# AllenInstitute/distributed-vae

Measured on AMD Instinct MI355X. Metric: cells/sec per train step (fwd+loss+bwd+opt), higher is better.
Workload: dtype f32; 1 GPU; cpl_mixVAE A=2 arms, synthetic-10x-v1 50000 cells x 5000 genes per GPU, batch 5000/GPU, fp32, H=100 L=10 C=92 S=2, x_drop=0.5, Adam lr=1e-3; global_batch=5000, parallelism=dp1, noise=in-kernel Philox4x32-10

## Files before the change

### distributed-vae_amd/_native.py

```python
from __future__ import annotations

import ctypes as C
import os
from typing import Dict, Optional

import torch

HERE = os.path.dirname(os.path.abspath(__file__))
LIB_PATH = os.environ.get("MMVAE_LIB") or os.path.join(HERE, "libmmvae_hip.so")

ABI_VERSION = 5
N_PARAM_TENSORS = 28
N_BN = 6
MAX_ARMS = 8

PARAM_NAMES = [
    "fc1.weight", "fc1.bias", "fc2.weight", "fc2.bias", "fc3.weight", "fc3.bias", "fc4.weight", "fc4.bias",
    "fc5.weight", "fc5.bias", "fcc.weight", "fcc.bias", "fc_mu.weight", "fc_sigma.weight", "fc_mu.bias",
    "fc_sigma.bias", "fc6.weight", "fc6.bias", "fc7.weight", "fc7.bias", "fc8.weight", "fc8.bias",
    "fc9.weight", "fc9.bias", "fc10.weight", "fc10.bias", "fc11.weight", "fc11.bias",
]
BN_NAMES = ["batch_l1", "batch_l2", "batch_l3", "batch_l4", "batch_l5", "batch_s"]

WS_IDS = {name: i for i, name in enumerate([
# ... 81 lines not shown
    "fc11": ("FC11_GENERAL", "FC11_ZG", "FC11_ZT", "FC11_BF16", "FC11_X3", "FC11_OUT_BF16", "FC11_OUT_X3"),
    "zero": ("ZERO_NONE", "ZERO_MEMSET", "ZERO_XBITS", "ZERO_PRESPLIT"),
    "couple": ("COUPLE_INLINE", "COUPLE_SIDE", "COUPLE_IN_DEC"),
}


def debug_plan(dims: "Dims", hyper: "Hyper", ex: Optional["Exec"], kind: str, params_align: int = 16, x_align: int = 16,
               x_arm_stride: int = 0, has_x16: bool = False, fc11_grad: bool = True) -> Dict[str, object]:
    out = (C.c_int32 * PLAN_FIELDS)()
    check(lib().mmvae_debug_plan(C.byref(dims), C.byref(hyper), C.byref(ex) if ex is not None else None, CALL_KINDS[kind],
                                 int(params_align), int(x_align), int(x_arm_stride), int(bool(has_x16)), int(bool(fc11_grad)),
                                 C.byref(out)), "mmvae_debug_plan")
    plan = {}
    for name, v in zip(PLAN_NAMES, out):
        if name in PLAN_ENUMS:
            plan[name] = PLAN_ENUMS[name][v]
        elif name == "kind":
            plan[name] = next(k for k, i in CALL_KINDS.items() if i == v)
        elif name in ("gd10_slabs", "dw11_slabs"):
            plan[name] = int(v)
        else:
            plan[name] = bool(v)
    return plan


_lib = None


def lib():
    global _lib
    if _lib is not None:
        return _lib
    if not os.path.exists(LIB_PATH):
        raise NativeError(
            f"{LIB_PATH} not found: build the HIP extension first "
            "(python -c 'import __graft_entry__ as g; g.build()' or python distributed-vae_amd/build.py). "
            "There is no CPU fallback.")
    L = C.CDLL(LIB_PATH)
    vp, i64, f32, i32 = C.c_void_p, C.c_int64, C.c_float, C.c_int
    L.mmvae_abi_version.restype = C.c_int
    L.mmvae_last_error_string.restype = C.c_char_p
    L.mmvae_check_dims.argtypes = [C.POINTER(Dims)]
    L.mmvae_param_layout.argtypes = [C.POINTER(Dims), C.POINTER(ParamLayout)]
    ex = C.POINTER(Exec)
    L.mmvae_workspace_bytes.argtypes = [C.POINTER(Dims), ex]
    L.mmvae_workspace_bytes.restype = C.c_size_t
    L.mmvae_ws_offset.argtypes = [C.POINTER(Dims), ex, C.c_int]
    L.mmvae_ws_offset.restype = i64
    L.mmvae_splits.argtypes = [C.POINTER(Dims), ex, C.POINTER(C.c_int32 * 6)]
    L.mmvae_forward.argtypes = [C.POINTER(Dims), C.POINTER(Hyper), C.POINTER(Noise), vp, vp, vp, vp, i64, vp, i32,
                                vp, C.c_size_t, ex, vp]
    L.mmvae_loss.argtypes = [C.POINTER(Dims), C.POINTER(Hyper), vp, C.c_size_t, vp, ex, vp]
    L.mmvae_backward.argtypes = [C.POINTER(Dims), C.POINTER(Hyper), C.POINTER(Noise), vp, vp, i64, f32, vp,
                                 C.c_size_t, vp, ex, vp]
    L.mmvae_adam_step.argtypes = [i64, vp, vp, vp, vp, i64, f32, f32, f32, f32, f32, i32, vp]
    L.mmvae_train_step.argtypes = [C.POINTER(Dims), C.POINTER(Hyper), C.POINTER(Noise), vp, vp, vp, vp, i64, vp,
                                   C.c_size_t, vp, vp, i32, vp, vp, i64, f32, f32, f32, f32, f32, i32, ex, vp]
    L.mmvae_train_step_rows.argtypes = [C.POINTER(Dims), C.POINTER(Hyper), C.POINTER(Noise), vp, vp, vp, vp, vp, i64, i64, vp, vp,
                                        C.c_size_t, vp, vp, i32, vp, vp, i64, f32, f32, f32, f32, f32, i32, ex, vp]
    L.mmvae_train_step_rows.restype = C.c_int
    L.mmvae_to_bf16.argtypes = [vp, i64, i64, i32, vp, vp]
    L.mmvae_to_bf16.restype = C.c_int
    L.mmvae_debug_stage.argtypes = [C.POINTER(Dims), C.POINTER(Hyper), C.POINTER(Noise), i32, vp, vp, i64, vp,
                                    C.c_size_t, vp, ex, vp]
    L.mmvae_dump_noise.argtypes = [C.POINTER(Dims), C.POINTER(Hyper), C.POINTER(Noise), vp, vp, vp, vp, vp]
    L.mmvae_debug_plan.argtypes = [C.POINTER(Dims), C.POINTER(Hyper), ex, i32, i32, i32, i64, i32, i32,
                                   C.POINTER(C.c_int32 * PLAN_FIELDS)]
    L.mmvae_debug_plan.restype = C.c_int
    L.mmvae_eval_classify.argtypes = [C.POINTER(Dims), C.POINTER(Hyper), vp, vp, vp, i64, vp, C.c_size_t, vp, vp, ex,
                                      vp]
    L.mmvae_classify.argtypes = [vp, i64, i32, vp, vp]
    L.mmvae_confmat_accumulate.argtypes = [vp, i32, i64, i32, vp, vp]
    L.mmvae_consensus.argtypes = [vp, i32, i32, vp, vp, vp]
    L.mmvae_aug_packed_floats.argtypes = [C.POINTER(AugDims)]
    L.mmvae_aug_packed_floats.restype = C.c_size_t
    L.mmvae_aug_workspace_bytes.argtypes = [C.POINTER(AugDims), i32]
    L.mmvae_aug_workspace_bytes.restype = C.c_size_t
    L.mmvae_aug_pack.argtypes = [C.POINTER(AugDims), C.POINTER(AugTensors), vp, vp]
    L.mmvae_augment.argtypes = [C.POINTER(AugDims), vp, vp, i64, vp, vp, f32, vp, C.c_size_t, vp, vp, i32, ex, vp]
    L.mmvae_gather_rows.argtypes = [vp, i64, i64, vp, i64, i32, vp, vp]
    L.mmvae_tp_planes_bytes.argtypes = [i64, i32, i32]
    L.mmvae_tp_planes_bytes.restype = C.c_size_t
    L.mmvae_tp_planes.argtypes = [vp, i64, i64, i32, i32, vp, vp]
    L.mmvae_augment_rows.argtypes = [C.POINTER(AugDims), vp, vp, i64, i32, vp, vp, vp, f32, vp, C.c_size_t, vp, vp, i32, ex, vp]
    L.mmvae_decode_workspace_bytes.argtypes = [C.POINTER(Dims), ex]
    L.mmvae_decode_workspace_bytes.restype = C.c_size_t
    L.mmvae_decode.argtypes = [C.POINTER(Dims), C.POINTER(Hyper), vp, vp, i64, vp, i64, vp, vp, C.c_size_t, ex, vp]
    L.mmvae_decode.restype = C.c_int
    L.mmvae_state_changes_workspace_bytes.argtypes = [C.POINTER(Dims), i32, ex]
    L.mmvae_state_changes_workspace_bytes.restype = C.c_size_t
    L.mmvae_state_changes.argtypes = [C.POINTER(Dims), C.POINTER(Hyper), C.POINTER(Noise), vp, vp, vp, i32, i32, vp, vp,
# ... 330 lines not shown
```

### distributed-vae_amd/csrc/api.hip

```cpp
#include "common.hpp"
#include <stdarg.h>
#include <stdio.h>
#include <string.h>

namespace mmvae {

static thread_local char g_err[512] = "";
void set_error(const char* fmt, ...) {
    va_list ap;
    va_start(ap, fmt);
    vsnprintf(g_err, sizeof(g_err), fmt, ap);
    va_end(ap);
}

Splits default_splits(const mmvae_dims& d, const mmvae_exec* ex) {
    int g_split[6] = {0, 0, 0, 0, 0, 0};
    if (ex) for (int i = 0; i < 6; ++i) g_split[i] = ex->split[i] > 0 && ex->split[i] <= 64 ? ex->split[i] : 0;
    constexpr int CUS = 256;
    auto fit = [](int base_blocks, int slots, int cap) {
        const int base = base_blocks > 0 ? base_blocks : 1;
        auto eff = [&](int k) { const int n = base * k; return (double)n / (double)(((n + slots - 1) / slots) * slots); };
        int pick = 1;
        double best = 0.0;
        for (int k = 1; k <= cap; ++k) {
// ... 19 lines not shown
    s.ks_small = g_split[3] > 0 ? g_split[3] : fit(N_SMALL * d.A, 3 * CUS, 32);
    s.ks_small = min(s.ks_small, max(1, cdiv(d.B, 32)));
    s.ks_gd10 = g_split[4] > 0 ? g_split[4] : fit(nb128 * d.A, (fastdims && d.H == 100 ? 2 : 3) * CUS, 16);
    if (g_split[4] <= 0 && fastdims && d.H == 100) {
        const int wg = cdiv(d.B, 256) * d.A;
        int best = s.ks_gd10;
        double best_eff = 0.0;
        for (int ks = 1; ks <= 16; ++ks) {
            const int n = wg * ks;
            const double eff = (double)n / (double)(cdiv(n, CUS) * CUS);
            if (eff > best_eff + 0.02) { best_eff = eff; best = ks; }
            if (eff >= 0.93) { best = ks; break; }
        }
        s.ks_gd10 = best;
    }
    s.ks_gd10 = min(s.ks_gd10, max(1, cdiv(d.D, fastdims && d.H == 100 ? 64 : 32)));
    if (ex && ex->tune[MMVAE_TUNE_ENGINE] == 2 && fastdims && x3_fc11_fits(d)) {
        const int pairs_b = cdiv(nb128, 2), pairs_d = cdiv(cdiv(d.D, 128), 2);
        if (g_split[0] <= 0) s.ks_fc1 = min(fit(pairs_b * d.A, CUS, 16), max(1, cdiv(d.D, 32)));
        if (g_split[4] <= 0) s.ks_gd10 = min(fit(nb128 * d.A, CUS, 16), max(1, cdiv(d.D, 64)));
        if (g_split[2] <= 0) s.ks_dw = min(fit(pairs_d * d.A, CUS, 16), max(1, cdiv(d.B, 32)));
        if (g_split[5] <= 0) {
            const int nwg = max(1, pairs_d * d.A);
            const bool chain_x3 = chain_planes_fit(d) && !ex->tune[MMVAE_TUNE_CHAIN_FP32];
            const int target = chain_x3 ? 140 : 3 * CUS / 8;
            s.ks_dw11 = min(max(1, (target + nwg / 2) / nwg), max(1, cdiv(d.B, 32)));
        }
        if (g_split[3] <= 0) s.ks_small = min(fit(cdiv(N_SMALL * d.A, 2), CUS, 32), max(1, cdiv(d.B, 32)));
    }
    if (ex && ex->tune[MMVAE_TUNE_ENGINE] == 1 && fastdims && bf16_tiles_fit(d)) {
        if (g_split[3] <= 0) s.ks_small = min(fit(cdiv(N_SMALL * d.A, 2), CUS, 32), max(1, cdiv(d.B, 32)));
        if (g_split[5] <= 0) {
            const int nwg = max(1, cdiv(d.D, 128) * d.A);
            s.ks_dw11 = min(max(1, (5 * CUS / 8 + nwg / 2) / nwg), max(1, cdiv(d.B, 32)));
        }
    }
    return s;
}

POff make_poff(const mmvae_dims& d) {
    POff p{};
    const int64_t D = d.D, H = d.H, L = d.L, C = d.C, S = d.S;
    const int64_t sizes[MMVAE_N_PARAM_TENSORS] = {
        H * D, H, H * H, H, H * H, H, H * H, H, L * H, L, C * L, C, S * (L + C), S * (L + C), S, S,
        L * (C + S), L, H * L, H, H * H, H, H * H, H, H * H, H, D * H, D};
    int64_t off = 0;
    for (int t = 0; t < MMVAE_N_PARAM_TENSORS; ++t) {
// ... 152 lines not shown
static void make_plan(Ctx& c, CallKind kind, const float* params, const float* x, int64_t xs, bool fc11_grad = true) {
    const mmvae_dims& d = c.d;
    const mmvae_hyper& h = c.h;
    const Layout& L = c.lay;
    Plan& p = c.plan;
    p = Plan{};
    p.kind = kind;
    const bool step = kind == CALL_STEP || kind == CALL_STEP_ROWS, fwd = step || kind == CALL_FORWARD || kind == CALL_CLASSIFY ||
                                                                 kind == CALL_TRAVERSE;
    const bool dropout = c.dropout(), side = c.side() != nullptr;
    p.fast = fast_dims(d) && al16(params) && al16(x) && (xs & 3) == 0 && d.H >= 4 && (int64_t)d.B * d.D < ((int64_t)1 << 30);
    const bool bf16_tiles = (h.gemm_bf16 == 1 || h.gemm_bf16 == 2) && bf16_tiles_fit(d);
    const bool x3 = h.gemm_bf16 == 2 && bf16_tiles_fit(d);
    p.big = !p.fast ? GEMM_GENERAL : x3 ? GEMM_X3 : bf16_tiles ? GEMM_BF16 : GEMM_FP32;
    p.small_x3 = bf16_tiles;
    const bool slots = fc11_slots_fit(L, d.B);
    if (!p.fast) p.fc11 = FC11_GENERAL;
    else if (p.big == GEMM_X3 && fc11_grad && x3_fc11_fits(d) && slots) p.fc11 = FC11_X3;
    else if (p.big == GEMM_BF16) p.fc11 = FC11_BF16;
    else if (fc11_grad && d.H == 100 && (int64_t)cdiv(d.B, 256) * L.sp.ks_gd10 <= L.n11) p.fc11 = FC11_ZG;
    else p.fc11 = FC11_ZT;
    p.gd10_slabs = p.fast ? L.sp.ks_gd10 : L.sp.ns_fc11;
    p.dw11_slabs = p.fast ? L.sp.ks_dw11 : L.sp.ks_dw;
    p.chain_planes = p.fast && bf16_tiles && chain_planes_fit(d) && !c.tune(MMVAE_TUNE_CHAIN_FP32);
    p.lat_half = d.C <= 32 * LH_CPL && d.L <= 32 && 2 * d.S <= 32;
    p.narrow = h.gemm_bf16 == 1 && c.x16 != nullptr && bf16_tiles_fit(d) && (d.D & 7) == 0;
    p.presplit = fwd && p.fast && (x3 || p.chain_planes);
    p.bwd_small_planes = kind == CALL_BACKWARD && p.chain_planes;
    p.d10_planes = x3;
    p.dz1_in_apply = (x3 || p.narrow) && (d.H & 1) == 0;
    if (fwd && h.training) p.zero = p.presplit && dropout ? ZERO_PRESPLIT : p.fast && dropout ? ZERO_XBITS : ZERO_MEMSET;
    p.rowmap = kind == CALL_STEP_ROWS && p.zero == ZERO_PRESPLIT && slots && (p.fc11 == FC11_X3 || p.fc11 == FC11_BF16);
    p.dz11_bf16 = p.rowmap && c.x16 != nullptr && p.fc11 == FC11_BF16;
    p.dw11_side = (step || kind == CALL_BACKWARD) && p.fast && side;
    p.loss_on_side = step && p.fast && side;
    const int cs = c.tune(MMVAE_TUNE_COUPLE_SIDE);
    const bool role = p.loss_on_side && c.use_acc() && p.chain_planes && d.A >= 2 && d.A <= 5 && cs != 1 && (d.A >= 4 || cs == 3);
    p.couple = step && side ? (role ? COUPLE_IN_DEC : COUPLE_SIDE) : COUPLE_INLINE;
    p.lat_fork_rides = p.couple == COUPLE_SIDE && p.lat_half;
    p.fc11_fork_rides = p.loss_on_side && (p.fc11 == FC11_X3 || p.fc11 == FC11_BF16);
    if (kind == CALL_DECODE) {
        if (!p.fast) p.fc11 = FC11_GENERAL;
        else if (p.big == GEMM_X3 && x3_fc11_fits(d)) p.fc11 = FC11_OUT_X3;
        else if (p.big == GEMM_BF16) p.fc11 = FC11_OUT_BF16;
        else p.fc11 = FC11_ZT;
        p.d10_planes = p.fc11 == FC11_OUT_X3 || p.fc11 == FC11_OUT_BF16;
        p.dec_planes = p.d10_planes || p.chain_planes;
    }
}

static int fork_to_side(const Ctx& c, int ev, bool rode = false) {
// ... 456 lines not shown
            if (!fast) return launch_dw_big(c, nz, x, x_arm_stride);
            if (int rc = dw1(c, x, x_arm_stride)) return rc;
            return dw11(c);
        case 9: return launch_make_xbits(c, nz);
        case 20: return launch_chain_fwd_enc(c, 3, params, nullptr, nullptr);
        case 21: return launch_chain_bwd_enc(c, 3, params);
        case 10: case 11: case 12: case 13: case 14:
            if (!fast) { set_error("stage %d needs the fast path", stage); return MMVAE_E_UNSUPPORTED; }
            if (stage == 10) return fc11_main(c, params, x, x_arm_stride, nullptr, 1);
            if (stage == 11) return fc11_gd10(c, params, nullptr, 1);
            if (stage == 12) return dw1(c, x, x_arm_stride);
            if (stage == 13) return dw11(c);
            return fc1_gemm(c, params, x, x_arm_stride);
        case 3: return launch_dw_small(c);
        case 4: return launch_chain_fwd_dec(c, params);
        case 5: return launch_chain_bwd_dec(c, params);
        case 6: return launch_lat_fwd(c, nz, params, nullptr, nullptr);
        case 7: return launch_lat_bwd(c, nz, params);
        case 8: if (!grads) { set_error("grads is null"); return MMVAE_E_BADARG; } return launch_reduce_grads(c, grads, 1.f, nullptr);
        default: set_error("unknown stage %d", stage); return MMVAE_E_BADARG;
    }
}

int mmvae_debug_plan(const mmvae_dims* d, const mmvae_hyper* h, const mmvae_exec* ex, int call_kind, int params_align,
                     int x_align, int64_t x_arm_stride, int has_x16, int fc11_grad, int32_t out[MMVAE_PLAN_FIELDS]) {
    if (int rc = check_dims(d)) return rc;
    if (!h || !out) { set_error("null hyper / out"); return MMVAE_E_BADARG; }
    if (int rc = check_gemm_engine(h->gemm_bf16)) return rc;
    static_assert(MMVAE_CALL_STEP == CALL_STEP && MMVAE_CALL_STEP_ROWS == CALL_STEP_ROWS && MMVAE_CALL_FORWARD == CALL_FORWARD &&
                  MMVAE_CALL_BACKWARD == CALL_BACKWARD && MMVAE_CALL_LOSS == CALL_LOSS && MMVAE_CALL_CLASSIFY == CALL_CLASSIFY &&
                  MMVAE_CALL_REPLAY == CALL_REPLAY && MMVAE_CALL_DECODE == CALL_DECODE && MMVAE_CALL_TRAVERSE == CALL_TRAVERSE,
                  "MMVAE_CALL_* (include/mmvae.h) are the values of CallKind");
    if (call_kind < CALL_STEP || call_kind > CALL_TRAVERSE) { set_error("unknown call kind %d", call_kind); return MMVAE_E_BADARG; }
    if (params_align < 0 || x_align < 0) { set_error("negative alignment"); return MMVAE_E_BADARG; }
    Ctx c{};
    c.d = *d;
    c.h = *h;
    if (call_kind == CALL_DECODE || call_kind == CALL_TRAVERSE || call_kind == CALL_CLASSIFY) c.h.training = 0;
    if (ex) c.ex = *ex; else memset(&c.ex, 0, sizeof(c.ex));
    c.lay = make_layout(*d, &c.ex);
    c.po = make_poff(*d);
    const uintptr_t base = 1u << 20;
    const float* params = reinterpret_cast<const float*>(base + (uintptr_t)(params_align & 15));
    const float* x = reinterpret_cast<const float*>(2 * base + (uintptr_t)(x_align & 15));
    if (has_x16 && call_kind == CALL_STEP_ROWS) c.x16 = reinterpret_cast<const unsigned short*>(3 * base);
    make_plan(c, (CallKind)call_kind, params, x, x_arm_stride, fc11_grad != 0);
    const Plan& p = c.plan;
    const int32_t v[] = {(int32_t)p.kind, p.fast, (int32_t)p.big, p.small_x3, (int32_t)p.fc11, p.gd10_slabs, p.dw11_slabs, p.chain_planes,
                         p.lat_half, p.narrow, p.presplit, p.bwd_small_planes, p.d10_planes, p.dz1_in_apply, p.dec_planes,
                         (int32_t)p.zero, p.rowmap, p.dz11_bf16, p.dw11_side, p.loss_on_side, (int32_t)p.couple, p.lat_fork_rides,
                         p.fc11_fork_rides};
    static_assert(sizeof(v) / sizeof(v[0]) == MMVAE_PLAN_FIELDS, "one value per field of Plan, in declaration order");
    for (int i = 0; i < MMVAE_PLAN_FIELDS; ++i) out[i] = v[i];
    return 0;
}

int mmvae_dump_noise(const mmvae_dims* d, const mmvae_hyper* h, const mmvae_noise* nz, uint8_t* x_mask,
                     float* u_gumbel, float* u_state, uint8_t* s_mask, void* stream) {
    if (int rc = check_dims(d)) return rc;
    if (!h || !nz) { set_error("null hyper / noise"); return MMVAE_E_BADARG; }
    return launch_dump_noise(*d, *h, nz, x_mask, u_gumbel, u_state, s_mask, reinterpret_cast<hipStream_t>(stream));
}

}
```

### distributed-vae_amd/csrc/chain.hip

```cpp
#include "common.hpp"
#include "couple.hpp"
#include <stdlib.h>
#include <type_traits>

namespace mmvae {

constexpr int CH_RT = CHAIN_ROWS / 32;
constexpr int CH_NT = 256 * CH_RT;

struct FwdLayer {
    int64_t w_off, b_off;
    int64_t out_off;
    int K, N, act;
    int64_t obn_mean_off = -1, obn_rstd_off = -1;
    int pl_slot = -1;
};
struct ChainFwdArgs {
    int nlayers;
    FwdLayer L[5];
    int64_t x_off;
    int K0;
    int64_t bn_mean_off, bn_rstd_off;
    int64_t bn_part_off;
    int part_n, part_rows;
// ... 681 lines not shown
                    s2 += __shfl_xor(s2, 32, 64);
                    ps1[ti] = s1;
                    ps2[ti] = s2;
                }
            }
        }
        if (last && a.part_off >= 0) {
#pragma unroll
            for (int ti = 0; ti < NTI; ++ti) {
                const int col = (ct + 4 * ti) * 32 + (lane & 31);
                if (lane < 32) { Ws[(rt * 2 + 0) * 256 + col] = ps1[ti]; Ws[(rt * 2 + 1) * 256 + col] = ps2[ti]; }
            }
            lds_barrier();
            if (tid < K) {
                float t1 = 0.f, t2 = 0.f;
#pragma unroll
                for (int k = 0; k < CH_RT; ++k) { t1 += Ws[(k * 2 + 0) * 256 + tid]; t2 += Ws[(k * 2 + 1) * 256 + tid]; }
                if (a.acc_out_off >= 0) {
                    acc_add_sums(reinterpret_cast<long long*>(ws + a.acc_out_off) + (int64_t)arm * ACC_SET_I64, tid, t1, t2);
                } else {
                    float* p = ws + a.part_off + (((int64_t)arm * gridDim.x + blk) * 2) * K;
                    p[tid] = t1;
                    p[K + tid] = t2;
                }
            }
        }
        lds_barrier();
    }
}

__global__ __launch_bounds__(256) void k_bn_bwd_apply(const float* __restrict__ G, const float* __restrict__ R,
                                                      const float* __restrict__ mean, const float* __restrict__ rstd,
                                                      const float* __restrict__ part, int npart,
                                                      const long long* __restrict__ acc, float* __restrict__ DZ,
                                                      int B, int W, unsigned short* __restrict__ planes, int Rp) {
    __shared__ __attribute__((aligned(16))) double scratch[1024];
    __shared__ float sums_s[2][128], mu_s[128], rs_s[128];
    const int arm = blockIdx.y, blk = blockIdx.x, tid = threadIdx.x;
    if (acc) {
        if (tid < W) {
            double s1, s2;
            acc_get(acc + (int64_t)arm * ACC_SET_I64, tid, s1, s2);
            sums_s[0][tid] = (float)s1;
            sums_s[1][tid] = (float)s2;
        }
    } else {
// ... 194 lines not shown
    ChainBwdArgs a{};
    a.nlayers = 5;
    a.L[0] = BwdLayer{c.po.o[24], L.DZ[10], L.Dk[4], d.H, d.H};
    a.L[1] = BwdLayer{c.po.o[22], L.DZ[9], L.Dk[3], d.H, d.H};
    a.L[2] = BwdLayer{c.po.o[20], L.DZ[8], L.Dk[2], d.H, d.H};
    a.L[3] = BwdLayer{c.po.o[18], L.DZ[7], L.Dk[1], d.L, d.H};
    a.L[4] = BwdLayer{c.po.o[16], L.DZ[6], L.Dk[0], d.C + d.S, d.L};
    a.g_off = L.GD10_slab;
    a.nslab = c.plan.gd10_slabs;
    a.slab_stride = (int64_t)d.A * d.B * d.H;
    a.bnb_part_off = -1;
    a.bn_mean_off = a.bn_rstd_off = -1;
    a.gout_off = L.GZIN;
    a.part_off = -1;
    a.rprev_off = a.rprev_mean_off = a.rprev_rstd_off = -1;
    a.acc_in_off = a.acc_out_off = -1;
    a.zero_off = acc_set_off(L, d.A, ACC_BWD);
    a.zero_n4 = c.use_acc() ? (int)(c.bwd_zero_floats() / 4) : 0;
    a.B = d.B;
    a.ld = bwd_ld(max(max(d.H, d.L), d.C + d.S));
    a.wrows = max(rup(max(d.H, d.L), 8), cdiv(WS_SCRATCH, a.ld));
    a.per_arm = c.po.per_arm;
    for (int i = 0; i < 5; ++i) a.L[i].pl_slot = PL_SMALL_LAYERS + 8 - i;
    return launch_bwd(c, a, max(max(d.H, d.L), d.C + d.S), params, "k_chain_bwd<dec>");
}

int launch_chain_bwd_enc(const Ctx& c, int layer, const float* params) {
    const mmvae_dims& d = c.d;
    const Layout& L = c.lay;
    ChainBwdArgs a{};
    a.nlayers = 1;
    const int i = layer - 1;
    const int N = (layer == 5) ? d.L : d.H;
    a.L[0] = BwdLayer{c.po.o[2 * (layer - 1)], L.DZ[layer], L.R[i], d.H, N};
    a.g_off = L.G[layer];
    a.nslab = 1;
    a.slab_stride = 0;
    a.bnb_part_off = L.bnb_part[layer];
    a.bnb_n = (layer == 5) ? cdiv(d.B, LAT_ROWS_BWD) : L.nblkc;
    a.bn_mean_off = L.bn_mean[i];
    a.bn_rstd_off = L.bn_rstd[i];
    a.gout_off = L.G[layer - 1];
    a.part_off = L.bnb_part[layer - 1];
    a.rprev_off = L.R[i - 1];
    a.rprev_mean_off = L.bn_mean[i - 1];
    a.rprev_rstd_off = L.bn_rstd[i - 1];
// ... 27 lines not shown
```

### distributed-vae_amd/csrc/common.hpp

```cpp
#pragma once
#include <hip/hip_runtime.h>
#include <hip/hip_ext.h>
#include <stdint.h>
#include "../../include/mmvae.h"
#include "tune.h"

namespace mmvae {

typedef float f32x16 __attribute__((ext_vector_type(16)));

constexpr int WAVE = 64;
constexpr int ROWS32 = 32;
constexpr int NP = 128;
constexpr int MAP_PAD = 256;
constexpr int DW11_LD = 132;
constexpr int SMALL_LD = 256;

__host__ __device__ inline int cdiv(int a, int b) { return (a + b - 1) / b; }
__host__ __device__ inline int64_t cdiv64(int64_t a, int64_t b) { return (a + b - 1) / b; }
__host__ __device__ inline int rup(int a, int b) { return cdiv(a, b) * b; }
__host__ __device__ inline int64_t imin64(int64_t a, int64_t b) { return a < b ? a : b; }

struct Splits {
    int ks_fc1;
// ... 605 lines not shown
    CallKind kind;
    bool fast;
    GemmFamily big;
    bool small_x3;
    Fc11Family fc11;
    int gd10_slabs;
    int dw11_slabs;
    bool chain_planes;
    bool lat_half;
    bool narrow;
    bool presplit;
    bool bwd_small_planes;
    bool d10_planes;
    bool dz1_in_apply;
    bool dec_planes;
    FwdZero zero;
    bool rowmap;
    bool dz11_bf16;
    bool dw11_side;
    bool loss_on_side;
    CouplePlace couple;
    bool lat_fork_rides;
    bool fc11_fork_rides;
};

struct Ctx {
    mmvae_dims d;
    mmvae_hyper h;
    Layout lay;
    POff po;
    float* ws;
    hipStream_t stream;
    mmvae_exec ex;
    mmvae_exec* ex_out;
    hipStream_t side() const { return reinterpret_cast<hipStream_t>(ex.side_stream); }
    hipEvent_t ev(int i) const { return reinterpret_cast<hipEvent_t>(ex.ev[i]); }
    int tune(int i) const { return ex.tune[i]; }
    bool use_acc() const { return !ex.tune[MMVAE_TUNE_BN_PARTIALS]; }
    bool dropout() const { return h.training && h.x_drop > 0.f; }
    float fc11_coef() const { return (float)(d.A > 1 ? d.A - 1 : 1) / (float)d.B; }
    int64_t fwd_zero_floats() const { return acc_set_off(lay, d.A, ACC_BWD) - lay.fc11_part; }
    int64_t bwd_zero_floats() const { return lay.acc_end - acc_set_off(lay, d.A, ACC_BWD); }
    const int64_t* x_rows = nullptr;
    const unsigned short* x16 = nullptr;
    int64_t x_ld = 0, x_nrows = 0;
    Plan plan{};
// ... 107 lines not shown
```

### distributed-vae_amd/csrc/gemm_bf16.hip

```cpp
#include "common.hpp"

namespace mmvae {

typedef __bf16 bf16x8 __attribute__((ext_vector_type(8)));
typedef __bf16 bf16x2 __attribute__((ext_vector_type(2)));
typedef unsigned int u32x4v __attribute__((ext_vector_type(4)));


constexpr int BT = 128;
constexpr int KT = 64;
constexpr int LDB = 36;
constexpr int LDK = 136;

template <int NP>
struct Eng {
    static constexpr int KT = NP == 1 ? 64 : 32;
    static constexpr int NQ = KT / 8;
    static constexpr int LDB = KT / 2 + 4;
    static constexpr int PLANE = BT * LDB;
    static constexpr int LDK = NP == 1 ? 136 : 160;
    static constexpr int NBUF = NP == 1 ? 2 : 1;
};

__device__ __forceinline__ unsigned pack_bf16(float a, float b) {
// ... 309 lines not shown
template <bool KMINOR>
__device__ __forceinline__ void plane_load(PlaneRegs& t, const PlaneDev& o, int r0, int k0, int j) {
    const int tid = threadIdx.x & 255, pl = j >> 1, id = tid + 256 * (j & 1);
    int off;
    if (!KMINOR) off = pl * o.plane + (r0 + (id >> 2)) * o.ld + k0 + 8 * (id & 3);
    else off = pl * o.plane + (k0 + (id >> 4)) * o.ld + r0 + 8 * (id & 15);
    t.v[j] = __builtin_bit_cast(u32x4v, __builtin_amdgcn_raw_buffer_load_b128(o.rs, off * 2, 0, 0));
}
template <bool KMINOR>
__device__ __forceinline__ void plane_store(unsigned* __restrict__ T, const PlaneRegs& t, int j) {
    const int tid = threadIdx.x & 255, pl = j >> 1, id = tid + 256 * (j & 1);
    int idx;
    if (!KMINOR) idx = pl * Eng<3>::PLANE + (id >> 2) * Eng<3>::LDB + 4 * (id & 3);
    else idx = pl * Eng<3>::PLANE + (((id >> 4) * Eng<3>::LDK + 8 * (id & 15)) >> 1);
    *reinterpret_cast<u32x4v*>(&T[idx]) = t.v[j];
}

struct SplitJob {
    const float* src; int64_t ld, src_arm;
    int R, C, Rp, Cp, ones_col;
    unsigned short* dst; int64_t dst_arm;
    const float* col_src; int64_t col_arm;
    int tr;
};
struct XbitsJob {
    NoiseDev nz; int A, B, D, wpr; uint32_t* bits; int blocks; float* zero_p; int zero_n4;
    const int64_t* rows; unsigned* map; int64_t rows_ld, n_rows;
};
struct SplitJobs { SplitJob j[24]; int first[25]; int n; XbitsJob xb; };
__global__ __launch_bounds__(256) void k_presplit(const SplitJobs js) {
    if (js.xb.zero_n4 > 0) grid_zero(js.xb.zero_p, js.xb.zero_n4);
    if (js.xb.rows && blockIdx.z == 0) {
        for (int i = blockIdx.x * 256 + threadIdx.x; i < js.xb.B + MAP_PAD; i += gridDim.x * 256) {
            const int64_t r = i < js.xb.B ? js.xb.rows[i] : 0;
            js.xb.map[i] = (unsigned)((r < 0 ? 0 : (r >= js.xb.n_rows ? js.xb.n_rows - 1 : r)) * js.xb.rows_ld);
        }
    }
    if ((int)blockIdx.x < js.xb.blocks) {
        make_xbits_range(js.xb.nz, js.xb.A, js.xb.B, js.xb.D, js.xb.wpr, js.xb.bits,
                         ((int64_t)blockIdx.z * js.xb.blocks + blockIdx.x) * 256 + threadIdx.x, (int64_t)gridDim.z * js.xb.blocks * 256);
        return;
    }
    const int bx0 = (int)blockIdx.x - js.xb.blocks;
    int ji = 0;
    while (ji + 1 < js.n && bx0 >= js.first[ji + 1]) ++ji;
    const SplitJob& J = js.j[ji];
// ... 6 lines not shown
    const bool vec = (J.ld & 3) == 0 && (J.C & 3) == 0;
    const int n = J.Rp * c8n;
    for (int i = bx * 256 + threadIdx.x; i < n; i += nbx * 256) {
        const int r = i / c8n, c0 = (i - r * c8n) * 8;
        float v[8];
        if (J.tr) {
#pragma unroll
            for (int e = 0; e < 8; ++e) v[e] = (r < J.R && c0 + e < J.C) ? src[(int64_t)(c0 + e) * J.ld + r] : 0.f;
        } else if (r < J.R && vec && c0 + 8 <= J.C) {
            const float4 a = *reinterpret_cast<const float4*>(src + (int64_t)r * J.ld + c0);
            const float4 b = *reinterpret_cast<const float4*>(src + (int64_t)r * J.ld + c0 + 4);
            v[0] = a.x; v[1] = a.y; v[2] = a.z; v[3] = a.w; v[4] = b.x; v[5] = b.y; v[6] = b.z; v[7] = b.w;
        } else {
#pragma unroll
            for (int e = 0; e < 8; ++e) {
                const int c = c0 + e;
                v[e] = (r < J.R && c < J.C) ? src[(int64_t)r * J.ld + c] : ((r < J.R && c == J.ones_col) ? (col ? col[r] : 1.f) : 0.f);
            }
        }
        unsigned w[4][3];
#pragma unroll
        for (int e = 0; e < 4; ++e) split3(v[2 * e], v[2 * e + 1], w[e]);
#pragma unroll
        for (int pl = 0; pl < 3; ++pl)
            *reinterpret_cast<uint4*>(dst + pl * plane + (int64_t)r * J.Cp + c0) = make_uint4(w[0][pl], w[1][pl], w[2][pl], w[3][pl]);
    }
}

struct SlabOut {
    float* out;
    int64_t ks_stride, arm_stride;
    int ld, M, N;
};
struct Fc11Out {
    const float* bias;
    const float* x;
    float* dz;
    float* x_rec;
    float* part;
    float coef;
    int B, D;
    const unsigned* xmap;
    int64_t x_nrec;
};

struct GemmArgs {
    Operand a, b;
    int64_t a_arm, b_arm;
// ... 1043 lines not shown
    return SplitJob{src, ld, src_arm, g.R, g.C, g.Rp, g.Cp, g.ones_col, reinterpret_cast<unsigned short*>(c.ws + g.ws_off),
                    3 * (int64_t)g.Rp * g.Cp, col_src, col_arm};
}
static int launch_presplit(hipStream_t s, int A, const SplitJob* jobs, int n, const XbitsJob* xb = nullptr) {
    SplitJobs js{};
    if (xb) js.xb = *xb;
    js.n = n;
    for (int i = 0; i < n; ++i) {
        js.j[i] = jobs[i];
        js.first[i + 1] = js.first[i] + (int)imin64(1024, cdiv64((int64_t)jobs[i].Rp * (jobs[i].Cp / 8), 256));
    }
    hipLaunchKernelGGL(k_presplit, dim3(js.xb.blocks + js.first[n], 1, A), dim3(256), 0, s, js);
    HIP_LAUNCH_CHECK("k_presplit");
    return 0;
}

static SplitJob small_plane_job(const Ctx& c, const float* params, int s, bool transposed) {
    const int H = c.d.H, L = c.d.L, CS = c.d.C + c.d.S;
    const int ti[PL_SMALL_LAYERS] = {2, 4, 6, 8, 16, 18, 20, 22, 24};
    const int nn[PL_SMALL_LAYERS] = {H, H, H, L, L, H, H, H, H}, kk[PL_SMALL_LAYERS] = {H, H, H, H, CS, L, H, H, H};
    unsigned short* base = reinterpret_cast<unsigned short*>(c.ws + c.lay.pl_small);
    return SplitJob{params + c.po.o[ti[s]], kk[s], c.po.per_arm, transposed ? kk[s] : nn[s], transposed ? nn[s] : kk[s], 128, 128, -1,
                    base + (int64_t)(transposed ? PL_SMALL_LAYERS + s : s) * 3 * 128 * 128, (int64_t)PL_SMALL_SLOTS * 3 * 128 * 128,
                    nullptr, 0, transposed ? 1 : 0};
}

int launch_x3_planes(const Ctx& c, const float* params, bool head, const mmvae_noise* nz) {
    const Plan& p = c.plan;
    const mmvae_dims& d = c.d;
    XbitsJob xb{};
    const bool xbits = head && p.zero == ZERO_PRESPLIT;
    if (xbits) {
        xb.nz = make_noise_dev(nz, c.h);
        xb.A = d.A; xb.B = d.B; xb.D = d.D; xb.wpr = cdiv(d.D, 32);
        xb.bits = reinterpret_cast<uint32_t*>(c.ws + c.lay.xbits);
        xb.blocks = (int)imin64(2048, cdiv64((int64_t)d.B * cdiv(xb.wpr, xbits_words_per_thread(xb.nz)), 256));
        xb.zero_p = c.ws + c.lay.fc11_part;
        xb.zero_n4 = (int)(c.fwd_zero_floats() / 4);
        if (p.rowmap) {
            xb.rows = c.x_rows; xb.map = reinterpret_cast<unsigned*>(c.ws + c.lay.rowmap);
            xb.rows_ld = c.x_ld; xb.n_rows = c.x_nrows;
        }
    }
    SplitJob jobs[24];
    int n = 0;
    if (head && (p.big == GEMM_X3 || p.narrow)) {
        jobs[n++] = plane_job(c, PL_W1, params + c.po.o[0], d.D, c.po.per_arm);
// ... 214 lines not shown
```

### include/mmvae.h

```cpp
#ifndef MMVAE_H
#define MMVAE_H

#include <stddef.h>
#include <stdint.h>

#ifdef __cplusplus
extern "C" {
#endif

#define MMVAE_OK 0
#define MMVAE_E_BADARG (-1)
#define MMVAE_E_UNSUPPORTED (-2)
#define MMVAE_E_LAUNCH (-3)
#define MMVAE_E_WORKSPACE (-4)

#define MMVAE_MAX_ARMS 8
#define MMVAE_N_PARAM_TENSORS 28
#define MMVAE_N_BN 6

typedef struct mmvae_dims {
    int32_t A, B, D, H, L, C, S;
} mmvae_dims;

typedef struct mmvae_hyper {
// ... 177 lines not shown
                        mmvae_exec *ex, void *stream);

int mmvae_dump_noise(const mmvae_dims *d, const mmvae_hyper *h, const mmvae_noise *nz,
                     uint8_t *x_mask, float *u_gumbel, float *u_state, uint8_t *s_mask,
                     void *stream);

int mmvae_debug_stage(const mmvae_dims *d, const mmvae_hyper *h, const mmvae_noise *nz, int stage,
                      const float *params, const float *x, int64_t x_arm_stride, void *ws,
                      size_t ws_bytes, float *grads, mmvae_exec *ex, void *stream);

#define MMVAE_PLAN_FIELDS 23
#define MMVAE_CALL_STEP 0
#define MMVAE_CALL_STEP_ROWS 1
#define MMVAE_CALL_FORWARD 2
#define MMVAE_CALL_BACKWARD 3
#define MMVAE_CALL_LOSS 4
#define MMVAE_CALL_CLASSIFY 5
#define MMVAE_CALL_REPLAY 6
#define MMVAE_CALL_DECODE 7
#define MMVAE_CALL_TRAVERSE 8
int mmvae_debug_plan(const mmvae_dims *d, const mmvae_hyper *h, const mmvae_exec *ex, int call_kind,
                     int params_align, int x_align, int64_t x_arm_stride, int has_x16, int fc11_grad,
                     int32_t out[MMVAE_PLAN_FIELDS]);

#ifdef __cplusplus
}
#endif
#endif
```

Baseline: 7.459 million cells/s.

## Add 32-row decoder backward chain kernel with register-resident pre-fragmented weights

Adds k_chain_bwd32, a decoder backward chain kernel that handles 32 rows per block. It keeps bf16x3 weight fragments in registers, loaded from a new fragment-ordered plane layout written by the presplit kernel, and prefetches the next layer's weights during the current MFMA. The goal is more blocks across the CUs for B=5000 and fewer LDS weight loads in the small-layer backward chain. The path is on by default for training steps when chain planes apply. A tune value of 2 disables it, and a debug entry point reports which row count was picked. The cost is higher register pressure, plus a layout coupling between presplit and the new kernel.

```diff
diff --git a/distributed-vae_amd/_native.py b/distributed-vae_amd/_native.py
--- a/distributed-vae_amd/_native.py
+++ b/distributed-vae_amd/_native.py
@@ -127,6 +127,16 @@
         else:
             plan[name] = bool(v)
     return plan
+
+
+def debug_dec_bwd_cells(dims: "Dims", hyper: "Hyper", ex: Optional["Exec"], kind: str, params_align: int = 16, x_align: int = 16,
+                        x_arm_stride: int = 0, has_x16: bool = False, fc11_grad: bool = True) -> int:
+    rc = lib().mmvae_debug_dec_bwd_cells(C.byref(dims), C.byref(hyper), C.byref(ex) if ex is not None else None, CALL_KINDS[kind],
+                                         int(params_align), int(x_align), int(x_arm_stride), int(bool(has_x16)),
+                                         int(bool(fc11_grad)))
+    if rc < 0:
+        check(rc, "mmvae_debug_dec_bwd_cells")
+    return rc
 
 
 _lib = None
@@ -172,6 +182,9 @@
     L.mmvae_debug_plan.argtypes = [C.POINTER(Dims), C.POINTER(Hyper), ex, i32, i32, i32, i64, i32, i32,
                                    C.POINTER(C.c_int32 * PLAN_FIELDS)]
     L.mmvae_debug_plan.restype = C.c_int
+    if hasattr(L, "mmvae_debug_dec_bwd_cells"):
+        L.mmvae_debug_dec_bwd_cells.argtypes = [C.POINTER(Dims), C.POINTER(Hyper), ex, i32, i32, i32, i64, i32, i32]
+        L.mmvae_debug_dec_bwd_cells.restype = C.c_int
     L.mmvae_eval_classify.argtypes = [C.POINTER(Dims), C.POINTER(Hyper), vp, vp, vp, i64, vp, C.c_size_t, vp, vp, ex,
                                       vp]
     L.mmvae_classify.argtypes = [vp, i64, i32, vp, vp]
diff --git a/distributed-vae_amd/csrc/api.hip b/distributed-vae_amd/csrc/api.hip
--- a/distributed-vae_amd/csrc/api.hip
+++ b/distributed-vae_amd/csrc/api.hip
@@ -65,7 +65,7 @@
         if (g_split[2] <= 0) s.ks_dw = min(fit(pairs_d * d.A, CUS, 16), max(1, cdiv(d.B, 32)));
         if (g_split[5] <= 0) {
             const int nwg = max(1, pairs_d * d.A);
-            const bool chain_x3 = chain_planes_fit(d) && !ex->tune[MMVAE_TUNE_CHAIN_FP32];
+            const bool chain_x3 = chain_planes_fit(d) && ex->tune[MMVAE_TUNE_CHAIN_FP32] != 1;
             const int target = chain_x3 ? 140 : 3 * CUS / 8;
             s.ks_dw11 = min(max(1, (target + nwg / 2) / nwg), max(1, cdiv(d.B, 32)));
         }
@@ -264,11 +264,12 @@
     else p.fc11 = FC11_ZT;
     p.gd10_slabs = p.fast ? L.sp.ks_gd10 : L.sp.ns_fc11;
     p.dw11_slabs = p.fast ? L.sp.ks_dw11 : L.sp.ks_dw;
-    p.chain_planes = p.fast && bf16_tiles && chain_planes_fit(d) && !c.tune(MMVAE_TUNE_CHAIN_FP32);
+    p.chain_planes = p.fast && bf16_tiles && chain_planes_fit(d) && c.tune(MMVAE_TUNE_CHAIN_FP32) != 1;
     p.lat_half = d.C <= 32 * LH_CPL && d.L <= 32 && 2 * d.S <= 32;
     p.narrow = h.gemm_bf16 == 1 && c.x16 != nullptr && bf16_tiles_fit(d) && (d.D & 7) == 0;
     p.presplit = fwd && p.fast && (x3 || p.chain_planes);
     p.bwd_small_planes = kind == CALL_BACKWARD && p.chain_planes;
+    p.dec_bwd32 = step && p.chain_planes && c.tune(MMVAE_TUNE_CHAIN_FP32) != 2;
     p.d10_planes = x3;
     p.dz1_in_apply = (x3 || p.narrow) && (d.H & 1) == 0;
     if (fwd && h.training) p.zero = p.presplit && dropout ? ZERO_PRESPLIT : p.fast && dropout ? ZERO_XBITS : ZERO_MEMSET;
@@ -771,10 +772,10 @@
     }
 }
 
-int mmvae_debug_plan(const mmvae_dims* d, const mmvae_hyper* h, const mmvae_exec* ex, int call_kind, int params_align,
-                     int x_align, int64_t x_arm_stride, int has_x16, int fc11_grad, int32_t out[MMVAE_PLAN_FIELDS]) {
+static int debug_make_plan(Ctx& c, const mmvae_dims* d, const mmvae_hyper* h, const mmvae_exec* ex, int call_kind, int params_align,
+                           int x_align, int64_t x_arm_stride, int has_x16, int fc11_grad) {
     if (int rc = check_dims(d)) return rc;
-    if (!h || !out) { set_error("null hyper / out"); return MMVAE_E_BADARG; }
+    if (!h) { set_error("null hyper / out"); return MMVAE_E_BADARG; }
     if (int rc = check_gemm_engine(h->gemm_bf16)) return rc;
     static_assert(MMVAE_CALL_STEP == CALL_STEP && MMVAE_CALL_STEP_ROWS == CALL_STEP_ROWS && MMVAE_CALL_FORWARD == CALL_FORWARD &&
                   MMVAE_CALL_BACKWARD == CALL_BACKWARD && MMVAE_CALL_LOSS == CALL_LOSS && MMVAE_CALL_CLASSIFY == CALL_CLASSIFY &&
@@ -782,7 +783,6 @@
                   "MMVAE_CALL_* (include/mmvae.h) are the values of CallKind");
     if (call_kind < CALL_STEP || call_kind > CALL_TRAVERSE) { set_error("unknown call kind %d", call_kind); return MMVAE_E_BADARG; }
     if (params_align < 0 || x_align < 0) { set_error("negative alignment"); return MMVAE_E_BADARG; }
-    Ctx c{};
     c.d = *d;
     c.h = *h;
     if (call_kind == CALL_DECODE || call_kind == CALL_TRAVERSE || call_kind == CALL_CLASSIFY) c.h.training = 0;
@@ -794,14 +794,29 @@
     const float* x = reinterpret_cast<const float*>(2 * base + (uintptr_t)(x_align & 15));
     if (has_x16 && call_kind == CALL_STEP_ROWS) c.x16 = reinterpret_cast<const unsigned short*>(3 * base);
     make_plan(c, (CallKind)call_kind, params, x, x_arm_stride, fc11_grad != 0);
+    return 0;
+}
+
+int mmvae_debug_plan(const mmvae_dims* d, const mmvae_hyper* h, const mmvae_exec* ex, int call_kind, int params_align,
+                     int x_align, int64_t x_arm_stride, int has_x16, int fc11_grad, int32_t out[MMVAE_PLAN_FIELDS]) {
+    if (!out) { set_error("null hyper / out"); return MMVAE_E_BADARG; }
+    Ctx c{};
+    if (int rc = debug_make_plan(c, d, h, ex, call_kind, params_align, x_align, x_arm_stride, has_x16, fc11_grad)) return rc;
     const Plan& p = c.plan;
     const int32_t v[] = {(int32_t)p.kind, p.fast, (int32_t)p.big, p.small_x3, (int32_t)p.fc11, p.gd10_slabs, p.dw11_slabs, p.chain_planes,
                          p.lat_half, p.narrow, p.presplit, p.bwd_small_planes, p.d10_planes, p.dz1_in_apply, p.dec_planes,
                          (int32_t)p.zero, p.rowmap, p.dz11_bf16, p.dw11_side, p.loss_on_side, (int32_t)p.couple, p.lat_fork_rides,
                          p.fc11_fork_rides};
-    static_assert(sizeof(v) / sizeof(v[0]) == MMVAE_PLAN_FIELDS, "one value per field of Plan, in declaration order");
+    static_assert(sizeof(v) / sizeof(v[0]) == MMVAE_PLAN_FIELDS, "one value per read-back field of Plan, in declaration order");
     for (int i = 0; i < MMVAE_PLAN_FIELDS; ++i) out[i] = v[i];
     return 0;
+}
+
+int mmvae_debug_dec_bwd_cells(const mmvae_dims* d, const mmvae_hyper* h, const mmvae_exec* ex, int call_kind, int params_align,
+                              int x_align, int64_t x_arm_stride, int has_x16, int fc11_grad) {
+    Ctx c{};
+    if (int rc = debug_make_plan(c, d, h, ex, call_kind, params_align, x_align, x_arm_stride, has_x16, fc11_grad)) return rc;
+    return c.plan.dec_bwd32 ? 32 : CHAIN_ROWS;
 }
 
 int mmvae_dump_noise(const mmvae_dims* d, const mmvae_hyper* h, const mmvae_noise* nz, uint8_t* x_mask,
diff --git a/distributed-vae_amd/csrc/chain.hip b/distributed-vae_amd/csrc/chain.hip
--- a/distributed-vae_amd/csrc/chain.hip
+++ b/distributed-vae_amd/csrc/chain.hip
@@ -727,6 +727,181 @@
                     float* p = ws + a.part_off + (((int64_t)arm * gridDim.x + blk) * 2) * K;
                     p[tid] = t1;
                     p[K + tid] = t2;
+                }
+            }
+        }
+        lds_barrier();
+    }
+}
+
+constexpr int C32_ROWS = 32, C32_NT = 256, C32_KS = 8;
+__device__ __forceinline__ void wfrag_load(u32x4c (&wf)[3][C32_KS], const unsigned short* __restrict__ slot, int ct, int ksteps) {
+    const unsigned short* p = slot + ct * (3 * C32_KS * 512) + lane_id() * 8;
+#pragma unroll
+    for (int pl = 0; pl < 3; ++pl)
+#pragma unroll
+        for (int s = 0; s < C32_KS; ++s)
+            if (s < ksteps) wf[pl][s] = *reinterpret_cast<const u32x4c*>(p + (pl * C32_KS + s) * 512);
+}
+__device__ __forceinline__ void mma_x3_wfrag(f32x16& acc, const unsigned* Xp, int xpl, int ldp, const u32x4c (&wf)[3][C32_KS], int ksteps) {
+    const int lane = lane_id();
+    const unsigned* pa = Xp + (lane & 31) * ldp + 4 * (lane >> 5);
+    bf16x8c a[3];
+#pragma unroll
+    for (int pl = 0; pl < 3; ++pl) a[pl] = __builtin_bit_cast(bf16x8c, *reinterpret_cast<const u32x4c*>(pa + pl * xpl));
+#pragma unroll
+    for (int st = 0; st < C32_KS; ++st) {
+        if (st < ksteps) {
+            const int sn = (st + 1 < ksteps) ? st + 1 : st;
+            bf16x8c an[3], b[3];
+#pragma unroll
+            for (int pl = 0; pl < 3; ++pl) {
+                an[pl] = __builtin_bit_cast(bf16x8c, *reinterpret_cast<const u32x4c*>(pa + pl * xpl + 8 * sn));
+                b[pl] = __builtin_bit_cast(bf16x8c, wf[pl][st]);
+            }
+            acc = __builtin_amdgcn_mfma_f32_32x32x16_bf16(a[2], b[0], acc, 0, 0, 0);
+            acc = __builtin_amdgcn_mfma_f32_32x32x16_bf16(a[0], b[2], acc, 0, 0, 0);
+            acc = __builtin_amdgcn_mfma_f32_32x32x16_bf16(a[1], b[1], acc, 0, 0, 0);
+            acc = __builtin_amdgcn_mfma_f32_32x32x16_bf16(a[1], b[0], acc, 0, 0, 0);
+            acc = __builtin_amdgcn_mfma_f32_32x32x16_bf16(a[0], b[1], acc, 0, 0, 0);
+            acc = __builtin_amdgcn_mfma_f32_32x32x16_bf16(a[0], b[0], acc, 0, 0, 0);
+#pragma unroll
+            for (int pl = 0; pl < 3; ++pl) a[pl] = an[pl];
+        }
+    }
+}
+__global__ __launch_bounds__(C32_NT) void k_chain_bwd32(const ChainBwdArgs a_in, float* __restrict__ ws) {
+    const ChainBwdArgs a = a_in;
+    extern __shared__ __attribute__((aligned(16))) float smem[];
+    unsigned* const Gp = reinterpret_cast<unsigned*>(smem);
+    const int ld = a.ld, xpl = C32_ROWS * ld;
+    const int arm = blockIdx.y, b0 = blockIdx.x * C32_ROWS;
+    const int tid = threadIdx.x, lane = tid & 63, ct = __builtin_amdgcn_readfirstlane(tid >> 6);
+    const int B = a.B, nvalid = min(C32_ROWS, B - b0);
+    const unsigned short* const WPL = reinterpret_cast<const unsigned short*>(ws + a.wpl_off) + (int64_t)arm * PL_SMALL_SLOTS * 3 * PLS;
+    u32x4c wf[3][C32_KS];
+    if (a.zero_n4 > 0) grid_zero(ws + a.zero_off, a.zero_n4);
+    {
+        const BwdLayer L0 = a.L[0];
+        const int N = L0.N, c4n = rup(N, 16) >> 2;
+        const bool has_act = L0.act_off >= 0;
+        const float* G = ws + a.g_off + (int64_t)arm * B * N;
+        const float* act = has_act ? ws + L0.act_off + (int64_t)arm * B * N : G;
+        float* dz = ws + L0.dz_off + (int64_t)arm * B * N;
+        const bool vec = (N & 3) == 0;
+        const int part = tid & 7, row = tid >> 3;
+        const bool rok = row < nvalid;
+        auto stage_g = [&](auto tag) __attribute__((always_inline)) {
+            constexpr bool V = decltype(tag)::value;
+            float4 gq[4], avq[4];
+#pragma unroll
+            for (int j = 0; j < 4; ++j) {
+                const int col = (part + 8 * j) * 4;
+                float4 g = make_float4(0.f, 0.f, 0.f, 0.f);
+                auto add_slabs = [&](auto chunk) __attribute__((always_inline)) {
+                    constexpr int CHK = decltype(chunk)::value;
+                    for (int s0 = 0; s0 < a.nslab; s0 += CHK) {
+                        float4 t[CHK];
+#pragma unroll
+                        for (int sl = 0; sl < CHK; ++sl)
+                            t[sl] = ldg4_t<V>(G + (int64_t)min(s0 + sl, a.nslab - 1) * a.slab_stride, N, b0 + row, col, B, N);
+#pragma unroll
+                        for (int sl = 0; sl < CHK; ++sl) {
+                            const bool on = s0 + sl < a.nslab;
+                            g.x += on ? t[sl].x : 0.f; g.y += on ? t[sl].y : 0.f; g.z += on ? t[sl].z : 0.f; g.w += on ? t[sl].w : 0.f;
+                        }
+                    }
+                };
+                if (a.nslab == 1) g = ldg4_t<V>(G, N, b0 + row, col, B, N);
+                else if (a.nslab <= 4) add_slabs(std::integral_constant<int, 4>{});
+                else add_slabs(std::integral_constant<int, 16>{});
+                gq[j] = g;
+                avq[j] = ldg4_t<V>(act, N, b0 + row, col, B, N);
+            }
+            if (ct * 32 < rup(L0.K, 32)) wfrag_load(wf, WPL + (int64_t)L0.pl_slot * 3 * PLS, ct, rup(N, 16) >> 4);
+#pragma unroll
+            for (int j = 0; j < 4; ++j) {
+                const int c = part + 8 * j, col = c * 4;
+                const float4 g = gq[j], av = avq[j];
+                float4 v;
+                v.x = (rok && col < N && (!has_act || av.x > 0.f)) ? g.x : 0.f;
+                v.y = (rok && col + 1 < N && (!has_act || av.y > 0.f)) ? g.y : 0.f;
+                v.z = (rok && col + 2 < N && (!has_act || av.z > 0.f)) ? g.z : 0.f;
+                v.w = (rok && col + 3 < N && (!has_act || av.w > 0.f)) ? g.w : 0.f;
+                if (c < c4n) {
+                    unsigned w0[3], w1[3];
+                    split3(v.x, v.y, w0);
+                    split3(v.z, v.w, w1);
+#pragma unroll
+                    for (int pl = 0; pl < 3; ++pl) *reinterpret_cast<uint2*>(Gp + pl * xpl + row * ld + c * 2) = make_uint2(w0[pl], w1[pl]);
+                    if (rok) {
+                        float* o = dz + (int64_t)(b0 + row) * N + col;
+                        if (V && col + 3 < N) *reinterpret_cast<float4*>(o) = v;
+                        else {
+                            if (col < N) o[0] = v.x;
+                            if (col + 1 < N) o[1] = v.y;
+                            if (col + 2 < N) o[2] = v.z;
+                            if (col + 3 < N) o[3] = v.w;
+                        }
+                    }
+                }
+            }
+        };
+        if (vec) stage_g(VecTag{});
+        else stage_g(ScalarTag{});
+    }
+    lds_barrier();
+    const int col = ct * 32 + (lane & 31);
+    for (int l = 0; l < a.nlayers; ++l) {
+        const BwdLayer Lr = a.L[l];
+        const int K = Lr.K, N = Lr.N;
+        const bool last = (l + 1 == a.nlayers);
+        const bool active = ct * 32 < rup(K, 32);
+        float pre[16];
+        {
+            const float* src = nullptr;
+            if (!last) {
+                const BwdLayer Ln = a.L[l + 1];
+                src = Ln.act_off >= 0 ? ws + Ln.act_off + (int64_t)arm * B * K : nullptr;
+            }
+#pragma unroll
+            for (int r = 0; r < 16; ++r) {
+                const int row = acc_row(r, lane);
+                const bool ok = src && active && col < K && row < nvalid;
+                pre[r] = ok ? src[(int64_t)(b0 + row) * K + col] : 1.f;
+            }
+        }
+        f32x16 acc = zero16();
+        if (active) mma_x3_wfrag(acc, Gp, xpl, ld, wf, rup(N, 16) >> 4);
+        if (!last) {
+            const BwdLayer Ln = a.L[l + 1];
+            if (ct * 32 < rup(Ln.K, 32)) wfrag_load(wf, WPL + (int64_t)Ln.pl_slot * 3 * PLS, ct, rup(Ln.N, 16) >> 4);
+        }
+        lds_barrier();
+        if (active) {
+            if (!last) {
+                const BwdLayer Ln = a.L[l + 1];
+                float* dz = ws + Ln.dz_off + (int64_t)arm * B * K;
+#pragma unroll
+                for (int r = 0; r < 16; ++r) {
+                    const int row = acc_row(r, lane);
+                    const bool ok = col < K && row < nvalid;
+                    const float v = (ok && pre[r] > 0.f) ? acc[r] : 0.f;
+                    if (ok) dz[(int64_t)(b0 + row) * K + col] = v;
+                    const float nbv = __builtin_bit_cast(float, __builtin_amdgcn_update_dpp(0, __builtin_bit_cast(int, v), 0xF5, 0xF, 0xF, false));
+                    if (!(lane & 1) && col < rup(K, 16)) {
+                        unsigned w3[3];
+                        split3(v, nbv, w3);
+#pragma unroll
+                        for (int pl = 0; pl < 3; ++pl) Gp[pl * xpl + row * ld + (col >> 1)] = w3[pl];
+                    }
+                }
+            } else {
+                float* go = ws + a.gout_off + (int64_t)arm * B * K;
+#pragma unroll
+                for (int r = 0; r < 16; ++r) {
+                    const int row = acc_row(r, lane);
+                    if (col < K && row < nvalid) go[(int64_t)(b0 + row) * K + col] = acc[r];
                 }
             }
         }
@@ -967,6 +1142,13 @@
     a.wrows = max(rup(max(d.H, d.L), 8), cdiv(WS_SCRATCH, a.ld));
     a.per_arm = c.po.per_arm;
     for (int i = 0; i < 5; ++i) a.L[i].pl_slot = PL_SMALL_LAYERS + 8 - i;
+    if (c.plan.dec_bwd32) {
+        a.ld = x3_ld(max(max(d.H, d.L), d.C + d.S));
+        a.wpl_off = L.pl_small;
+        hipLaunchKernelGGL(k_chain_bwd32, dim3(L.nblk32, d.A), dim3(C32_NT), (size_t)3 * C32_ROWS * a.ld * sizeof(float), c.stream, a, c.ws);
+        HIP_LAUNCH_CHECK("k_chain_bwd32<dec>");
+        return 0;
+    }
     return launch_bwd(c, a, max(max(d.H, d.L), d.C + d.S), params, "k_chain_bwd<dec>");
 }
 
diff --git a/distributed-vae_amd/csrc/common.hpp b/distributed-vae_amd/csrc/common.hpp
--- a/distributed-vae_amd/csrc/common.hpp
+++ b/distributed-vae_amd/csrc/common.hpp
@@ -651,6 +651,7 @@
     CouplePlace couple;
     bool lat_fork_rides;
     bool fc11_fork_rides;
+    bool dec_bwd32;
 };
 
 struct Ctx {
diff --git a/distributed-vae_amd/csrc/gemm_bf16.hip b/distributed-vae_amd/csrc/gemm_bf16.hip
--- a/distributed-vae_amd/csrc/gemm_bf16.hip
+++ b/distributed-vae_amd/csrc/gemm_bf16.hip
@@ -355,6 +355,7 @@
     unsigned short* dst; int64_t dst_arm;
     const float* col_src; int64_t col_arm;
     int tr;
+    int frag;
 };
 struct XbitsJob {
     NoiseDev nz; int A, B, D, wpr; uint32_t* bits; int blocks; float* zero_p; int zero_n4;
@@ -407,8 +408,11 @@
 #pragma unroll
         for (int e = 0; e < 4; ++e) split3(v[2 * e], v[2 * e + 1], w[e]);
 #pragma unroll
-        for (int pl = 0; pl < 3; ++pl)
-            *reinterpret_cast<uint4*>(dst + pl * plane + (int64_t)r * J.Cp + c0) = make_uint4(w[0][pl], w[1][pl], w[2][pl], w[3][pl]);
+        for (int pl = 0; pl < 3; ++pl) {
+            const int64_t at = J.frag ? (int64_t)((((r >> 5) * 3 + pl) * 8 + (c0 >> 4)) * 512 + ((r & 31) + 32 * ((c0 >> 3) & 1)) * 8)
+                                      : pl * plane + (int64_t)r * J.Cp + c0;
+            *reinterpret_cast<uint4*>(dst + at) = make_uint4(w[0][pl], w[1][pl], w[2][pl], w[3][pl]);
+        }
     }
 }
 
@@ -1498,7 +1502,7 @@
     unsigned short* base = reinterpret_cast<unsigned short*>(c.ws + c.lay.pl_small);
     return SplitJob{params + c.po.o[ti[s]], kk[s], c.po.per_arm, transposed ? kk[s] : nn[s], transposed ? nn[s] : kk[s], 128, 128, -1,
                     base + (int64_t)(transposed ? PL_SMALL_LAYERS + s : s) * 3 * 128 * 128, (int64_t)PL_SMALL_SLOTS * 3 * 128 * 128,
-                    nullptr, 0, transposed ? 1 : 0};
+                    nullptr, 0, transposed ? 1 : 0, transposed && s >= PL_SMALL_DEC0 && c.plan.dec_bwd32 ? 1 : 0};
 }
 
 int launch_x3_planes(const Ctx& c, const float* params, bool head, const mmvae_noise* nz) {
diff --git a/include/mmvae.h b/include/mmvae.h
--- a/include/mmvae.h
+++ b/include/mmvae.h
@@ -223,6 +223,8 @@
 int mmvae_debug_plan(const mmvae_dims *d, const mmvae_hyper *h, const mmvae_exec *ex, int call_kind,
                      int params_align, int x_align, int64_t x_arm_stride, int has_x16, int fc11_grad,
                      int32_t out[MMVAE_PLAN_FIELDS]);
+int mmvae_debug_dec_bwd_cells(const mmvae_dims *d, const mmvae_hyper *h, const mmvae_exec *ex, int call_kind,
+                              int params_align, int x_align, int64_t x_arm_stride, int has_x16, int fc11_grad);
 
 #ifdef __cplusplus
 }
```

Result: slower. 7.208 million cells/s (-3.4%).
